# FurkanOM/tf-ssd

Hardware: AMD Instinct MI355X
Metric: images/sec SSD300 (MobileNetV2) fwd+NMS (higher is better)
Workload: dtype f32

## Files before the change

### tf-ssd_amd/csrc/ssd_conv.h

```cpp
#pragma once
#include "common.h"

namespace ssd {

struct ConvParams {
    const float* in;
    const float* w;
    const short* w3;
    const float* scale;
    const float* shift;
    const float* residual;
    float* out;
    int B, H, W, Cin, Ho, Wo, Cout;
    int kh, kw, stride, dil, pad_t, pad_l;
    int K, Kpad, Npad;
    long M;
    long out_batch_stride, out_pixel_stride;
    int n_split;
    float* out2;
    long out2_batch_stride, out2_pixel_stride;
    int vec_store2;
    int act;
    int vec_store;
    int split_k;
    float* partial;
    const float* wino_w;
    int bf16;
    const short* xp;
    long xp_plane;
    int xp_np;
    short* op;
    long op_plane;
    int op_np;
};
bool conv_config_allowed(int cfg, int precision);
inline int conv_vec_store(const ConvParams& p) {
    return (((uintptr_t)p.out & 15) == 0) && (p.out_pixel_stride % 4 == 0) && (p.out_batch_stride % 4 == 0);
}

struct FusedBlockParams {
    const float* x;
    float* y;
    const float* we;
    const float *es, *eh;
    const float* wd;
    const float *ds, *dh;
    const float* wp;
    const float *ps, *ph;
    int residual;
    int B, H, W, Cin, Ce, Cout, Ho, Wo, stride, pad_t, pad_l;
    int kpad_e, kpad_p, npad_p;
    int tiles_y, tiles_x;
    int bf16;
    int groups;
    const short* we3;
    const short* wp3;
    int bands;
    float* slabs;
    unsigned* tickets;
    float* e_out;
    short* y_planes;
    long y_plane;
    short* e_planes;
    long e_plane;
    int planes_np;
    int planes_only;
    int form2;
};
struct StemParams {
    const float* x;
    float* y;
    const float* w1;
    const float *s1, *h1;
    const float* wd;
    const float *sd, *hd;
    const float* wp;
    const float *sp, *hp;
    int B, H, W, H1, W1, pad_t, pad_l, kpad1, kpadp;
    int tiles_y, tiles_x;
    int bf16;
};
struct DwProjParams {
    const float* e;
    const float* wd;
    const float* dh;
    const float* wp;
    const float* ph;
    const float* res;
    float* y;
    int B, H, W, Ce, Cout, Ho, Wo, stride, pad_t, pad_l;
    int kpad_p, npad_p;
    int tiles_y, tiles_x;
    int bf16;
};
bool dwproj_supported(const DwProjParams& p);
int launch_dwproj(DwProjParams p, hipStream_t st);
bool stem_supported(const StemParams& p);
int launch_stem(StemParams p, hipStream_t st);
bool image_block2_supported(const FusedBlockParams& p);
int launch_image_block2(FusedBlockParams p, hipStream_t st);
bool fused_block_supported(const FusedBlockParams& p);
int launch_fused_block(FusedBlockParams p, hipStream_t st);
bool band3_block_supported(const FusedBlockParams& p);
size_t band3_we_shorts(int Ce);
size_t band3_wp_shorts(int npad_p, int Ce);
int launch_band3_pack(const float* we, int Ce, int Cin, int kpad_e, short* we3, const float* wp, int npad_p, int kpad_p,
                      short* wp3, hipStream_t st);
int launch_band3_block(FusedBlockParams p, hipStream_t st);
bool band_block_supported(const FusedBlockParams& p);
int launch_band_block(FusedBlockParams p, hipStream_t st);
bool image_block_supported(const FusedBlockParams& p);
bool image_block_split_fits(FusedBlockParams p);
int image_block_groups(const FusedBlockParams& p, int B);
size_t image_block_slab_floats(const FusedBlockParams& p, int B);
int launch_image_block(FusedBlockParams p, hipStream_t st);

inline int round_up(int v, int a) { return (v + a - 1) / a * a; }
inline int conv_kpad(int K) { return round_up(K, 32); }
inline int conv_npad(int Cout) { return round_up(Cout, 16); }

int conv_num_configs();
const char* conv_config_name(int cfg);
bool conv_config_valid(int cfg, const ConvParams& p);
int conv_pick_config(const ConvParams& p);
long conv_grid_blocks(int cfg, const ConvParams& p);
int conv_k_tiles(int cfg, const ConvParams& p);
int conv_launch(const ConvParams& p, int cfg, hipStream_t st);
size_t conv_splitk_workspace_floats(const ConvParams& p, int cfg);

int fill_conv_params(const ssd_conv_desc* d, ConvParams* p);
int launch_splitk_reduce(const ConvParams& p, hipStream_t st);

int conv_num_mfma_configs();
int wino_num_configs();
const char* wino_config_name(int i);
bool wino_applicable(const ConvParams& p);
bool wino_config_valid(int i, const ConvParams& p);
long wino_grid_blocks(int i, const ConvParams& p);
int wino_k_tiles(const ConvParams& p);
int wino_launch(const ConvParams& p, int i, hipStream_t st);
size_t wino_weight_floats(int Cin, int Cout);
int launch_wino_pack(const float* hwio, int Cin, int Cout, int Npad, int row_off, float* U, hipStream_t st);

int skinny_num_configs();
const char* skinny_config_name(int i);
bool skinny_config_valid(int i, const ConvParams& p);
long skinny_grid_blocks(int i, const ConvParams& p);
int skinny_launch(const ConvParams& p, int i, hipStream_t st);

int mfma3_num_configs();
const char* mfma3_config_name(int i);
bool mfma3_config_valid(int i, const ConvParams& p);
long mfma3_grid_blocks(int i, const ConvParams& p);
int mfma3_k_tiles(const ConvParams& p);
void mfma3_tile(int i, int* BM, int* BN);
int mfma3_launch(const ConvParams& p, int i, hipStream_t st, bool bf16 = false);
const char* bf16_config_name(int i);

int dma_num_configs();
const char* dma_config_name(int i, int np);
bool dma_config_valid(int i, int np, const ConvParams& p);
long dma_grid_blocks(int i, const ConvParams& p);
int dma_k_tiles(int np, const ConvParams& p);
// ... 35 lines not shown
```

### tf-ssd_amd/csrc/ssd_fused.hip

```cpp
#include <cstdlib>

#include "ssd_conv.h"
#include "ssd_bf16x3.h"
#include "ssd_block_common.h"

namespace ssd {

constexpr int kCK = 48;
constexpr int kLDE = kCK + 8;
constexpr int ldx_for(int cinp) { return cinp <= 24 ? 24 : cinp + 4; }

template <int NP, int CINP, int IW, int IPX>
__device__ __forceinline__ void expand_px_tiles(const float* Xs, const float* Wes, float* Es, const float* Ps,
                                                const int Ce, const int ce0, const int pt0, const int pt1,
                                                const int lane, const int iy0, const int ix0, const int H,
                                                const int W) {
    constexpr int LDX = ldx_for(CINP);
    const int frow = lane & 15, fk = (lane >> 4) * 4;
    const int pts[2] = {pt0, pt1};
    f32x4 ea[NP][3];
#pragma unroll
    for (int ct = 0; ct < 3; ++ct) {
        const f32x4 sh = *reinterpret_cast<const f32x4*>(Ps + Ce + ce0 + ct * 16 + (lane >> 4) * 4);
#pragma unroll
// ... 276 lines not shown
        }
    }
}

template <int CINP, int NTC, int S, int TH, int TW>
constexpr size_t fused_static_floats() {
    constexpr int IH = (TH - 1) * S + 3, IW = (TW - 1) * S + 3;
    constexpr int IPXP = (IH * IW + 15) / 16 * 16;
    return (size_t)IPXP * ldx_for(CINP) + (size_t)IPXP * kLDE + (size_t)TH * TW * kLDE + (size_t)kCK * ldx_for(CINP) +
           (size_t)NTC * 16 * kLDE;
}

typedef void (*fused_kernel_t)(const FusedBlockParams);

struct FusedCfg {
    int cinp, ntc, stride, th, tw, res;
    size_t static_floats;
    fused_kernel_t fn;
};
#define FCFG(CINP, NTC, S, TH, TW, RES)                                             \
    {CINP, NTC, S, TH, TW, RES, fused_static_floats<CINP, NTC, S, TH, TW>(),        \
     mbv2_block_kernel<CINP, NTC, S, TH, TW, RES != 0>}
static const FusedCfg kFused[] = {
    FCFG(16, 2, 2, 4, 8, 0),
    FCFG(24, 2, 1, 8, 8, 1),
    FCFG(24, 2, 2, 4, 8, 0),
    FCFG(32, 2, 1, 8, 8, 1),
    FCFG(32, 2, 1, 8, 8, 0),
    FCFG(32, 2, 2, 4, 8, 0),
    FCFG(32, 4, 2, 4, 8, 0),
    FCFG(32, 4, 1, 8, 8, 0),
    FCFG(32, 4, 1, 8, 8, 1),
};

static const FusedCfg* pick_fused(const FusedBlockParams& p) {
    if (p.Ce % kCK != 0 || p.Cin % 4 != 0 || p.Cout % 4 != 0 || p.e_out) return nullptr;
    const int cinp = p.Cin <= 16 ? 16 : (p.Cin == 24 ? 24 : (p.Cin <= 32 ? 32 : 0));
    const int ntc = p.Cout <= 32 ? 2 : (p.Cout <= 64 ? 4 : 0);
    if (!cinp || !ntc) return nullptr;
    for (const auto& c : kFused)
        if (c.cinp == cinp && c.ntc == ntc && c.stride == p.stride && c.res == (p.residual ? 1 : 0)) return &c;
    return nullptr;
}

bool fused_block_supported(const FusedBlockParams& p) { return pick_fused(p) != nullptr; }

int launch_fused_block(FusedBlockParams p, hipStream_t st) {
    const FusedCfg* c = pick_fused(p);
    if (!c) {
        set_error("fused block: unsupported shape Cin=%d Ce=%d Cout=%d stride=%d", p.Cin, p.Ce, p.Cout, p.stride);
        return SSD_E_UNSUPPORTED;
    }
    if (p.B == 0) return SSD_OK;
    p.tiles_y = (p.Ho + c->th - 1) / c->th;
    p.tiles_x = (p.Wo + c->tw - 1) / c->tw;
    const long tiles = (long)p.B * p.tiles_y * p.tiles_x;
    static int num_cu = 0;
    if (!num_cu) {
        int dev = 0;
        (void)hipGetDevice(&dev);
        if (hipDeviceGetAttribute(&num_cu, hipDeviceAttributeMultiprocessorCount, dev) != hipSuccess || num_cu <= 0)
            num_cu = 256;
    }
    constexpr int per_cu = 2;
    const long blocks = tiles < (long)per_cu * num_cu ? tiles : (long)per_cu * num_cu;
    const size_t lds = (c->static_floats + (size_t)13 * p.Ce + (size_t)2 * c->ntc * 16) * sizeof(float);
    SSD_UNSUPPORTED_IF(lds > 160 * 1024, "fused block: needs %zu B of LDS", lds);
    if (lds > 64 * 1024)
        SSD_HIP(hipFuncSetAttribute((const void*)c->fn, hipFuncAttributeMaxDynamicSharedMemorySize, (int)lds));
    hipLaunchKernelGGL(c->fn, dim3((unsigned)blocks), dim3(256), lds, st, p);
    SSD_LAUNCH_CHECK();
    return SSD_OK;
}

constexpr int kSTH = 8, kSTW = 16;
constexpr int kSIH = kSTH + 2, kSIW = kSTW + 2;
constexpr int kSPH = 2 * (kSIH - 1) + 3, kSPW = 2 * (kSIW - 1) + 3;
constexpr int kSLD = 40;
constexpr int kSPQ = (kSPW * 3 + 3 + 3) / 4, kSPR = kSPQ * 4;
constexpr int kSPS = (kSPH * kSPQ + 63) / 64 * 256;

template <bool DMA>
constexpr int stem_patch_floats() { return DMA ? 2 * kSPS : kSPH * kSPW * 3 + 5; }
template <bool DMA>
constexpr int stem_lds_floats() {
    return stem_patch_floats<DMA>() + kSIH * kSIW * kSLD + kSTH * kSTW * kSLD + 27 * 32 + 9 * 32 + 32 * 2 + 32 * 2 + 16 * 2;
}
template <int NP, bool DMA>
__device__ __forceinline__ void stem_body(const StemParams& p, float* __restrict__ sm) {
    static_assert(NP == 1 || NP == 3, "bf16 or split-bf16 operands");
    constexpr int RP = DMA ? kSPR : kSPW * 3;
    float* patch = sm;
    float* C1 = patch + stem_patch_floats<DMA>();
    float* D = C1 + kSIH * kSIW * kSLD;
    float* W1 = D + kSTH * kSTW * kSLD;
    float* Wd = W1 + 27 * 32;
    float* H1 = Wd + 9 * 32;
    float* Hd = H1 + 32;
    float* Hp = Hd + 32;

    const int tid = threadIdx.x, lane = tid & 63, wave = tid >> 6;
    int koff[2][4];
    int kcol[2][4];
    BP<NP> w1b[2], wpb;
    {
        f32x4 wl[2][2];
#pragma unroll
        for (int j = 0; j < 8; ++j) {
            const int k = (lane >> 4) * 8 + j;
            koff[j >> 2][j & 3] = k < 27 ? (k / 9) * RP + (k % 9) : 0;
            kcol[j >> 2][j & 3] = k < 27 ? k % 9 : 0;
#pragma unroll
            for (int ct = 0; ct < 2; ++ct) {
                const int ch = ct * 16 + (lane & 15);
                wl[ct][j >> 2][j & 3] = k < 27 ? p.w1[(long)ch * p.kpad1 + k] * p.s1[ch] : 0.f;
            }
        }
#pragma unroll
        for (int ct = 0; ct < 2; ++ct) w1b[ct] = splitN<NP>(wl[ct][0], wl[ct][1]);
        const int n = lane & 15;
        const float* wr = p.wp + (long)n * p.kpadp + (lane >> 4) * 8;
        f32x4 lo = *reinterpret_cast<const f32x4*>(wr), hi = *reinterpret_cast<const f32x4*>(wr + 4);
        wpb = splitN<NP>(lo * p.sp[n], hi * p.sp[n]);
    }
    for (int e = tid; e < 9 * 32; e += 256) Wd[e] = p.wd[e] * p.sd[e & 31];
    if (tid < 32) { H1[tid] = p.h1[tid]; Hd[tid] = p.hd[tid]; }
    if (tid < 16) Hp[tid] = p.hp[tid];

    const int tiles_per_img = p.tiles_y * p.tiles_x;
    const long total_tiles = (long)p.B * tiles_per_img;
    int du_row[3], du_q[3];
    if (DMA) {
#pragma unroll
        for (int j = 0; j < 3; ++j) {
            const int u = (wave + 4 * j) * 64 + lane;
            du_row[j] = u / kSPQ;
            du_q[j] = u - du_row[j] * kSPQ;
        }
    }
    auto tile_origin = [&](long tile, int& b, int& oy0, int& ox0, int& iy0, int& ix0) {
        b = (int)(tile / tiles_per_img);
        const int rem = (int)(tile - (long)b * tiles_per_img);
        const int ty = rem / p.tiles_x, tx = rem - ty * p.tiles_x;
        oy0 = ty * kSTH; ox0 = tx * kSTW;
        iy0 = (oy0 - 1) * 2 - p.pad_t; ix0 = (ox0 - 1) * 2 - p.pad_l;
    };
    auto issue_patch = [&](long tile, int stage) {
        if constexpr (DMA) {
            int b, oy0, ox0, iy0, ix0;
            tile_origin(tile, b, oy0, ox0, iy0, ix0);
            const __amdgpu_buffer_rsrc_t rs = __builtin_amdgcn_make_buffer_rsrc(const_cast<float*>(p.x + (long)b * p.H * p.W * 3), 0,
                                                                               p.H * p.W * 12, 0x00020000);
            const int fs = ((ix0 * 3) >> 2) * 4;
#pragma unroll
            for (int j = 0; j < 3; ++j) {
                const int ii = __builtin_amdgcn_readfirstlane(wave) + 4 * j;
                if (ii * 64 >= kSPH * kSPQ) continue;
                const int iy = iy0 + du_row[j];
                const bool ok = du_row[j] < kSPH && (unsigned)iy < (unsigned)p.H;
                const int off = ok ? (iy * p.W * 3 + fs + du_q[j] * 4) * 4 : (int)0x80000000;
                __builtin_amdgcn_raw_ptr_buffer_load_lds(rs, (lds_dst_t)(patch + stage * kSPS + ii * 256), 16, off, 0, 0, 0);
            }
        }
    };
    if (DMA && blockIdx.x < total_tiles) {
        issue_patch(blockIdx.x, 0);
        asm volatile("s_waitcnt vmcnt(0)" ::: "memory");
    }
    int it = 0;
    for (long tile = blockIdx.x; tile < total_tiles; tile += gridDim.x, ++it) {
        int b, oy0, ox0, iy0, ix0;
        tile_origin(tile, b, oy0, ox0, iy0, ix0);
        const int cy0 = oy0 - 1, cx0 = ox0 - 1;
        const float* img = p.x + (long)b * p.H * p.W * 3;
        const float* pbuf = patch;
        int psh = 0;

        __syncthreads();
        if constexpr (DMA) {
            pbuf = patch + (it & 1) * kSPS;
            psh = ix0 * 3 - ((ix0 * 3) >> 2) * 4;
            if (tile + gridDim.x < total_tiles) issue_patch(tile + gridDim.x, (it + 1) & 1);
        } else {
        {
            constexpr int NLD = (kSPH * kSPW * 3 + 255) / 256;
            float tmp[NLD];
#pragma unroll
            for (int i = 0; i < NLD; ++i) {
                const int e = tid + i * 256;
                const int r = e / (kSPW * 3), j = e - r * (kSPW * 3);
                const int iy = iy0 + r, ixc = ix0 * 3 + j;
                tmp[i] = 0.f;
                if (e < kSPH * kSPW * 3 && (unsigned)iy < (unsigned)p.H && ixc >= 0 && ixc < p.W * 3)
                    tmp[i] = img[(long)iy * p.W * 3 + ixc];
            }
#pragma unroll
            for (int i = 0; i < NLD; ++i) {
                const int e = tid + i * 256;
                if (e < kSPH * kSPW * 3) patch[e] = tmp[i];
            }
        }
        __syncthreads();
        }
        const int xlim = (p.W - ix0) * 3;
        const bool xedge = DMA && xlim < kSPW * 3;

        {
            constexpr int NHP = kSIH * kSIW;
            int hp[3], rr[3], cc[3];
            const float* pp[3];
            f32x4 a0[3], a1[3];
#pragma unroll
            for (int q = 0; q < 3; ++q) {
                hp[q] = (wave * 3 + q) * 16 + (lane & 15);
                const int hpc = hp[q] < NHP ? hp[q] : NHP - 1;
                rr[q] = hpc / kSIW;
                cc[q] = hpc - rr[q] * kSIW;
                pp[q] = pbuf + (2 * rr[q]) * RP + 2 * cc[q] * 3 + psh;
                a0[q] = *reinterpret_cast<const f32x4*>(H1 + (lane >> 4) * 4);
                a1[q] = *reinterpret_cast<const f32x4*>(H1 + 16 + (lane >> 4) * 4);
            }
#pragma unroll
            for (int q = 0; q < 3; ++q) {
                f32x4 lo, hi;
#pragma unroll
                for (int j = 0; j < 4; ++j) {
                    lo[j] = pp[q][koff[0][j]];
                    hi[j] = pp[q][koff[1][j]];
                }
                if (xedge) {
#pragma unroll
                    for (int j = 0; j < 4; ++j) {
                        if (cc[q] * 6 + kcol[0][j] >= xlim) lo[j] = 0.f;
                        if (cc[q] * 6 + kcol[1][j] >= xlim) hi[j] = 0.f;
                    }
                }
                const BP<NP> b = splitN<NP>(lo, hi);
                a0[q] = mmaN<NP>(w1b[0], b, a0[q]);
                a1[q] = mmaN<NP>(w1b[1], b, a1[q]);
            }
#pragma unroll
            for (int q = 0; q < 3; ++q) {
                const bool in = (unsigned)(cy0 + rr[q]) < (unsigned)p.H1 && (unsigned)(cx0 + cc[q]) < (unsigned)p.W1;
                const float hi = in ? 6.0f : 0.0f;
#pragma unroll
                for (int j = 0; j < 4; ++j) {
                    a0[q][j] = __builtin_amdgcn_fmed3f(a0[q][j], 0.0f, hi);
                    a1[q][j] = __builtin_amdgcn_fmed3f(a1[q][j], 0.0f, hi);
                }
                if (hp[q] < NHP) {
                    *reinterpret_cast<f32x4*>(C1 + hp[q] * kSLD + (lane >> 4) * 4) = a0[q];
                    *reinterpret_cast<f32x4*>(C1 + hp[q] * kSLD + 16 + (lane >> 4) * 4) = a1[q];
                }
            }
        }
        if constexpr (DMA) lds_barrier();
        else __syncthreads();

        {
            const int c4 = (tid & 7) * 4, strip = tid >> 3;
            const int oy = strip >> 2, ox = (strip & 3) * 4;
            f32x4 a[4];
            const f32x4 sh = *reinterpret_cast<const f32x4*>(Hd + c4);
#pragma unroll
            for (int t = 0; t < 4; ++t) a[t] = sh;
#pragma unroll
            for (int ky = 0; ky < 3; ++ky) {
                f32x4 e[6];
#pragma unroll
                for (int j = 0; j < 6; ++j) e[j] = *reinterpret_cast<const f32x4*>(C1 + ((oy + ky) * kSIW + ox + j) * kSLD + c4);
#pragma unroll
                for (int kx = 0; kx < 3; ++kx) {
                    const f32x4 w = *reinterpret_cast<const f32x4*>(Wd + (ky * 3 + kx) * 32 + c4);
#pragma unroll
                    for (int t = 0; t < 4; ++t) {
                        a[t] += e[t + kx] * w;
                    }
                }
            }
#pragma unroll
            for (int t = 0; t < 4; ++t) {
                f32x4 v = a[t];
#pragma unroll
                for (int j = 0; j < 4; ++j) v[j] = relu6f(v[j]);
                *reinterpret_cast<f32x4*>(D + (oy * kSTW + ox + t) * kSLD + c4) = v;
            }
        }
        if constexpr (DMA) lds_barrier();
        else __syncthreads();

        const int frow = lane & 15;
        f32x4 acc[2];
        acc[0] = acc[1] = *reinterpret_cast<const f32x4*>(Hp + (lane >> 4) * 4);
#pragma unroll
        for (int q = 0; q < 2; ++q) {
            const float* dr = D + ((wave + 4 * q) * 16 + frow) * kSLD + (lane >> 4) * 8;
            const BP<NP> b = splitN<NP>(*reinterpret_cast<const f32x4*>(dr), *reinterpret_cast<const f32x4*>(dr + 4));
            acc[q] = mmaN<NP>(wpb, b, acc[q]);
        }
        if constexpr (DMA) asm volatile("s_waitcnt vmcnt(0)" ::: "memory");
#pragma unroll
        for (int q = 0; q < 2; ++q) {
            const int po = (wave + 4 * q) * 16 + (lane & 15);
            const int oy = oy0 + po / kSTW, ox = ox0 + po % kSTW;
            if (oy < p.H1 && ox < p.W1)
                *reinterpret_cast<f32x4*>(p.y + (((long)b * p.H1 + oy) * p.W1 + ox) * 16 + (lane >> 4) * 4) = acc[q];
        }
    }
}

template <int NP, bool DMA>
__global__ __launch_bounds__(256) void mbv2_stem_kernel(const StemParams p) {
    __shared__ __attribute__((aligned(1024))) float sm[stem_lds_floats<DMA>()];
    stem_body<NP, DMA>(p, sm);
}

bool stem_supported(const StemParams& p) { return p.H1 >= 1 && p.W1 >= 1; }

int launch_stem(StemParams p, hipStream_t st) {
    if (p.B == 0) return SSD_OK;
    p.tiles_y = (p.H1 + kSTH - 1) / kSTH;
    p.tiles_x = (p.W1 + kSTW - 1) / kSTW;
    const long tiles = (long)p.B * p.tiles_y * p.tiles_x;
    const long blocks = tiles < 512 ? tiles : 512;
    const bool bf16 = p.bf16 == 1;
    const bool dma = p.W % 4 == 0 && (((uintptr_t)p.x) & 15) == 0 && (long)p.H * p.W * 12 < 0x7fffffffL;
    const auto fn = dma ? (bf16 ? mbv2_stem_kernel<1, true> : mbv2_stem_kernel<3, true>)
                        : (bf16 ? mbv2_stem_kernel<1, false> : mbv2_stem_kernel<3, false>);
    hipLaunchKernelGGL(fn, dim3((unsigned)blocks), dim3(256), 0, st, p);
    SSD_LAUNCH_CHECK();
    return SSD_OK;
}

}
```

### tf-ssd_amd/csrc/ssd_net.h

```cpp
#pragma once
#include <map>
#include <set>
#include <string>
#include <vector>

#include "ssd_conv.h"

struct ssd_train_state;
void ssd_train_state_free(ssd_train_state*);

namespace ssd {

enum LayerKind { LK_CONV = 0, LK_DW, LK_POOL, LK_L2NORM, LK_SOFTMAX, LK_FUSED };
static const char* kKindName[] = {"conv", "dw", "pool", "l2norm", "softmax", "fused"};

enum Route { RT_OFF = 0, RT_LAYER, RT_STEM, RT_DWPROJ, RT_TILE, RT_BAND, RT_BAND3, RT_IMAGE, RT_IMAGE_SPLIT };

struct Param {
    std::string name;
    std::vector<int> shape;
    size_t count = 0;
    float* dev = nullptr;
    bool set = false;
    bool in_flat = false;
// ... 17 lines not shown
    int in = -1, out = -1, res = -1;
    int H = 0, W = 0, Cin = 0, Ho = 0, Wo = 0, Cout = 0;
    int kh = 1, kw = 1, stride = 1, dil = 1, pt = 0, pl = 0, pb = 0, pr = 0, act = 0;
    int p_kernel = -1, p_bias = -1, p_bn = -1;
    int p_kernel2 = -1, p_bias2 = -1, Cout1 = 0;
    int p_gamma = -1;
    int head_kind = 0;
    long head_off = 0, head_bs = 0, head_ps = 0;
    long head2_off = 0, head2_bs = 0, head2_ps = 0;
    float* packed = nullptr;
    float* wino = nullptr;
    float* scale = nullptr;
    float* shift = nullptr;
    int cfg = -1;
    int split_k = 1;
    int f_expand = -1, f_dw = -1, f_project = -1;
    int f_type = 0;
    int fused_by = -1;
    int e_out = -1;
    int img_choice = -1;
    int fused_by2 = -1;
    Route route = RT_OFF;
    float* splitk_part = nullptr;
    float *fz_we = nullptr, *fz_wd = nullptr, *fz_wp = nullptr;
    float *fz_we3 = nullptr, *fz_wp3 = nullptr;
    int side = 0;
    hipEvent_t ev_ready = nullptr;
};

inline void conv_route_head(ConvParams& p, const Layer& l, float* probs, float* deltas) {
    p.out = probs + l.head_off;
    p.out_pixel_stride = l.head_ps;
    p.out_batch_stride = l.head_bs;
    p.n_split = l.Cout1;
    p.out2 = deltas + l.head2_off;
    p.out2_pixel_stride = l.head2_ps;
    p.out2_batch_stride = l.head2_bs;
    p.vec_store2 = (p.out2_pixel_stride % 4 == 0) && (p.out2_batch_stride % 4 == 0);
}

struct ScopedDev {
    float* p = nullptr;
    ~ScopedDev() { if (p) (void)hipFree(p); }
};
struct ScopedEvent {
    hipEvent_t e = nullptr;
    ~ScopedEvent() { if (e) (void)hipEventDestroy(e); }
};

struct Step {
    int layer = -1;
    int sid = -1;
    int wait[2] = {-1, -1};
    bool after_main = false;
    bool publishes = false;
    bool join_first = false;
};

}

struct ssd_net {
    int backbone = 0, img_size = 300, levels = 6, L = 21;
    std::vector<int> n_ars;
    std::vector<ssd::Param> params;
    std::map<std::string, int> param_index;
    std::vector<ssd::Tensor> tensors;
    std::map<std::string, int> tensor_index;
    std::vector<ssd::Layer> layers;
    std::vector<int> fmap;
    std::vector<long> level_off;
    int num_priors = 0;
    bool finalized = false;
    bool fuse_blocks = true;
    bool fuse_softmax = true;
    bool fuse_dwproj = true;
    bool use_wino = true;
    int precision = 0;
    int fuse_band = 2;
    int fuse_image = 1;
    int lanes_hint = 1;
    bool tail_on_side = false;
    bool image_split = true;
    bool image_v2 = true;
    bool conv_dma = true;
    bool plane_only = true;
    bool image_ticket = false;
    float* img_slabs = nullptr;
    unsigned* img_tickets = nullptr;
    int max_batch = 0;
    int last_batch = 0;
    std::vector<float*> owned;
    float* arena = nullptr;
    size_t arena_bytes = 0, plane_bytes = 0, slab_bytes = 0;
    float* splitk_ws = nullptr;
    size_t splitk_floats = 0;
    float* deltas = nullptr;
    float* probs = nullptr;
    void* nms_ws = nullptr;
    size_t nms_ws_bytes = 0;
    int nms_ws_batch = 0;
    int nms_ws_total = 0;
    int scratch_batch = 0;
    std::map<std::string, std::pair<std::string, int>> preset;
    int n_preset = 0;
    int n_autotuned = 0;
    bool launch_raced = false;
    bool use_graph = true;
    bool graphs_unsafe = false;
    bool use_graph_auto = true;
    struct GraphEntry {
        std::vector<const void*> key;
        hipGraphExec_t exec = nullptr;
        hipGraph_t graph = nullptr;
        const float* image = nullptr;
        int batch = 0;
    };
    std::vector<GraphEntry> graphs;
    hipStream_t gstream = nullptr;
    bool overlap_heads = true;
    static constexpr int kSides = 2;
    hipStream_t side[kSides] = {nullptr, nullptr};
    hipEvent_t ev_side_done[kSides] = {nullptr, nullptr};
    std::vector<ssd::Step> steps;
    float* splitk_layers = nullptr;
    bool timing = false;
    ssd_train_state* train = nullptr;
    std::set<std::string> frozen;
    unsigned trainable_rev = 0;
    std::vector<std::vector<hipEvent_t>> timing_events;

    ~ssd_net() {
        for (auto& p : params)
            if (p.dev && !p.in_flat) (void)hipFree(p.dev);
        if (train) ssd_train_state_free(train);
        for (float* p : owned)
            if (p) (void)hipFree(p);
        if (arena) (void)hipFree(arena);
        if (splitk_ws) (void)hipFree(splitk_ws);
        if (deltas) (void)hipFree(deltas);
        if (probs) (void)hipFree(probs);
        if (nms_ws) (void)hipFree(nms_ws);
        for (auto& v : timing_events)
            for (auto e : v) (void)hipEventDestroy(e);
        drop_graphs();
        if (gstream) (void)hipStreamDestroy(gstream);
        for (int k = 0; k < kSides; ++k) {
            if (side[k]) (void)hipStreamDestroy(side[k]);
            if (ev_side_done[k]) (void)hipEventDestroy(ev_side_done[k]);
        }
        for (auto& l : layers)
            if (l.ev_ready) (void)hipEventDestroy(l.ev_ready);
        if (splitk_layers) (void)hipFree(splitk_layers);
    }
    void drop_graphs() {
        steps.clear();
        for (auto& g : graphs) {
            if (g.exec) (void)hipGraphExecDestroy(g.exec);
            if (g.graph) (void)hipGraphDestroy(g.graph);
        }
        graphs.clear();
    }
};
```

### tf-ssd_amd/csrc/ssd_net.hip

```cpp
#include <algorithm>
#include <cstdlib>
#include <cstring>
#include <map>
#include <memory>
#include <string>
#include <vector>

#include "ssd_net.h"

using namespace ssd;

namespace ssd {

struct Builder {
    ssd_net& net;
    explicit Builder(ssd_net& n) : net(n) {}

    int add_param(const std::string& name, std::vector<int> shape) {
        Param p;
        p.name = name;
        p.shape = std::move(shape);
        p.count = 1;
        for (int d : p.shape) p.count *= (size_t)d;
        net.params.push_back(p);
// ... 293 lines not shown
    return p;
}

static FusedBlockParams fused_shape(const ssd_net& net, const Layer& f, int B) {
    const Layer& le = net.layers[f.f_expand];
    const Layer& ld = net.layers[f.f_dw];
    const Layer& lp = net.layers[f.f_project];
    FusedBlockParams p{};
    p.x = net.tensors[f.in].dev;
    p.y = net.tensors[f.out].dev;
    p.we = f.fz_we; p.es = le.scale; p.eh = le.shift;
    p.wd = f.fz_wd; p.ds = ld.scale; p.dh = ld.shift;
    p.wp = f.fz_wp; p.ps = lp.scale; p.ph = lp.shift;
    p.residual = lp.res >= 0 ? 1 : 0;
    p.B = B; p.H = f.H; p.W = f.W; p.Cin = f.Cin; p.Ce = le.Cout; p.Cout = f.Cout;
    p.Ho = f.Ho; p.Wo = f.Wo; p.stride = f.stride; p.pad_t = f.pt; p.pad_l = f.pl;
    p.kpad_e = conv_kpad(le.Cin);
    p.kpad_p = conv_kpad(lp.Cin);
    p.npad_p = conv_npad(lp.Cout);
    p.e_out = f.e_out >= 0 ? net.tensors[f.e_out].dev : nullptr;
    if (f.out >= 0 && net.tensors[f.out].planes_live) {
        const Tensor& to = net.tensors[f.out];
        p.y_planes = to.planes; p.y_plane = to.plane_stride; p.planes_np = to.planes_np;
    }
    if (f.e_out >= 0 && net.tensors[f.e_out].planes_live) {
        const Tensor& te = net.tensors[f.e_out];
        p.e_planes = te.planes; p.e_plane = te.plane_stride; p.planes_np = te.planes_np;
    }
    if (f.route == RT_IMAGE || f.route == RT_IMAGE_SPLIT)
        p.planes_only = (p.y_planes && net.tensors[f.out].plane_only ? 1 : 0) | (p.e_planes && net.tensors[f.e_out].plane_only ? 2 : 0);
    p.we3 = reinterpret_cast<const short*>(f.fz_we3);
    p.wp3 = reinterpret_cast<const short*>(f.fz_wp3);
    p.bf16 = net.precision;
    p.form2 = net.image_v2 ? 1 : 0;
    return p;
}

static FusedBlockParams fused_params(const ssd_net& net, const Layer& f, int B) {
    FusedBlockParams p = fused_shape(net, f, B);
    if (f.route == RT_IMAGE || f.route == RT_IMAGE_SPLIT) {
        const Layer& le = net.layers[f.f_expand];
        const Layer& lp = net.layers[f.f_project];
        p.we3 = conv_split_planes(f.fz_we, le.Cin, le.Cout);
        p.wp3 = conv_split_planes(f.fz_wp, lp.Cin, lp.Cout);
        p.groups = net.img_slabs ? image_block_groups(p, B * net.lanes_hint) : 1;
        p.slabs = net.img_slabs;
        p.tickets = net.image_ticket && !p.bf16 ? net.img_tickets : nullptr;
        if (f.route == RT_IMAGE_SPLIT) { p.bf16 = 3; p.tickets = nullptr; }
    }
    return p;
}

static DwProjParams dwproj_params(const ssd_net& net, const Layer& f, int B) {
    const Layer& ld = net.layers[f.f_dw];
    const Layer& lp = net.layers[f.f_project];
    DwProjParams p{};
    p.e = net.tensors[f.in].dev;
    p.y = net.tensors[f.out].dev;
    p.wd = f.fz_wd; p.dh = ld.shift;
    p.wp = f.fz_wp; p.ph = lp.shift;
    p.res = lp.res >= 0 ? net.tensors[lp.res].dev : nullptr;
    p.B = B; p.H = f.H; p.W = f.W; p.Ce = ld.Cout; p.Cout = f.Cout;
    p.Ho = f.Ho; p.Wo = f.Wo; p.stride = f.stride; p.pad_t = f.pt; p.pad_l = f.pl;
    p.kpad_p = conv_kpad(lp.Cin);
    p.npad_p = conv_npad(lp.Cout);
    p.bf16 = net.precision;
    return p;
}

static StemParams stem_params(const ssd_net& net, const Layer& f, int B) {
    const Layer& l1 = net.layers[f.f_expand];
    const Layer& ld = net.layers[f.f_dw];
    const Layer& lp = net.layers[f.f_project];
    StemParams p{};
    p.x = net.tensors[f.in].dev;
    p.y = net.tensors[f.out].dev;
    p.w1 = l1.packed; p.s1 = l1.scale; p.h1 = l1.shift;
    p.wd = net.params[ld.p_kernel].dev; p.sd = ld.scale; p.hd = ld.shift;
    p.wp = lp.packed; p.sp = lp.scale; p.hp = lp.shift;
    p.B = B; p.H = f.H; p.W = f.W; p.H1 = f.Ho; p.W1 = f.Wo; p.pad_t = f.pt; p.pad_l = f.pl;
    p.kpad1 = conv_kpad(27);
    p.kpadp = conv_kpad(32);
    p.bf16 = net.precision;
    return p;
}

static int planes_pass(ssd_net& net, int tensor, int B, hipStream_t st) {
    Tensor& t = net.tensors[tensor];
    return launch_split_planes(t.dev, (long)B * (long)t.per_image, t.C, t.planes_np, t.planes, t.plane_stride, st);
}

static int run_layer_kernels(ssd_net& net, const Layer& l, int B, float* deltas_out, float* probs_out, hipStream_t st,
                             int cfg_override) {
    const float* in = l.in >= 0 ? net.tensors[l.in].dev : nullptr;
    float* out = l.out >= 0 ? net.tensors[l.out].dev : nullptr;
    switch (l.kind) {
        case LK_CONV: {
            const float* res = l.res >= 0 ? net.tensors[l.res].dev : nullptr;
            ConvParams p = layer_conv_params(net, l, B, in, out, res, deltas_out, probs_out);
            const int cfg = cfg_override >= 0 ? cfg_override : l.cfg;
            const int rc = conv_launch(p, cfg, st);
            if (!rc && p.op && !conv_config_writes_planes(cfg, p)) return planes_pass(net, l.out, B, st);
            return rc;
        }
        case LK_DW:
            return launch_dwconv3x3(in, B, l.H, l.W, l.Cin, l.stride, l.pt, l.pl, l.Ho, l.Wo,
                                    net.params[l.p_kernel].dev, l.scale, l.shift, l.act, out, st);
        case LK_POOL: {
            const Tensor& to = net.tensors[l.out];
            return launch_maxpool(in, B, l.H, l.W, l.Cin, l.kh, l.stride, l.pt, l.pl, l.Ho, l.Wo, to.plane_only ? nullptr : out, st,
                                  to.planes_live ? to.planes : nullptr, to.plane_stride, to.planes_np);
        }
        case LK_L2NORM: {
            const Tensor& to = net.tensors[l.out];
            return launch_l2norm(in, (long)B * l.H * l.W, l.Cin, net.params[l.p_gamma].dev, to.plane_only ? nullptr : out, st,
                                 to.planes_live ? to.planes : nullptr, to.plane_stride, to.planes_np);
        }
        case LK_SOFTMAX:
            return launch_softmax(probs_out, (long)B * net.num_priors, net.L, probs_out, st);
        case LK_FUSED:
            switch (l.route) {
                case RT_STEM: return launch_stem(stem_params(net, l, B), st);
                case RT_DWPROJ: return launch_dwproj(dwproj_params(net, l, B), st);
                case RT_TILE: return launch_fused_block(fused_params(net, l, B), st);
                case RT_BAND: return launch_band_block(fused_params(net, l, B), st);
                case RT_BAND3: return launch_band3_block(fused_params(net, l, B), st);
                case RT_IMAGE:
                case RT_IMAGE_SPLIT: return launch_image_block(fused_params(net, l, B), st);
                default: break;
            }
            set_error("run_layer: no fused kernel is routed to layer %s", l.name.c_str());
            return SSD_E_STATE;
    }
    return SSD_OK;
}

static int run_layer_impl(ssd_net& net, const Layer& l, int B, float* deltas_out, float* probs_out, hipStream_t st,
                          int cfg_override) {
    int rc = run_layer_kernels(net, l, B, deltas_out, probs_out, st, cfg_override);
    if (rc || l.kind == LK_CONV || l.kind == LK_POOL || l.kind == LK_L2NORM || l.kind == LK_SOFTMAX) return rc;
    if ((l.route == RT_IMAGE || l.route == RT_IMAGE_SPLIT) && !net.image_ticket) return rc;
    if (l.out >= 0 && net.tensors[l.out].planes_live) rc = planes_pass(net, l.out, B, st);
    if (!rc && l.kind == LK_FUSED && l.e_out >= 0 && net.tensors[l.e_out].planes_live) rc = planes_pass(net, l.e_out, B, st);
    return rc;
}

static int run_layer(ssd_net& net, const Layer& l, int B, float* deltas_out, float* probs_out, hipStream_t st,
                     int cfg_override = -1) {
    static const bool dbg_sync = getenv("SSD_HIP_DEBUG_SYNC") != nullptr;
    if (!dbg_sync) return run_layer_impl(net, l, B, deltas_out, probs_out, st, cfg_override);
    fprintf(stderr, "[ssd dbg] run %s\n", l.name.c_str());
    const int rc = run_layer_impl(net, l, B, deltas_out, probs_out, st, cfg_override);
    hipStreamCaptureStatus cs = hipStreamCaptureStatusNone;
    (void)hipStreamIsCapturing(st, &cs);
    if (!rc && cs == hipStreamCaptureStatusNone) SSD_HIP(hipStreamSynchronize(st));
    return rc;
}

static bool image_kernel_takes(const FusedBlockParams& p) { return !fused_block_supported(p) && image_block_supported(p); }
static bool image_kernel_takes(const ssd_net& net, const Layer& f) {
    return f.kind == LK_FUSED && f.f_type == 0 && image_kernel_takes(fused_shape(net, f, 1));
}

static Route fused_route(const ssd_net& net, const Layer& f) {
    if (!net.fuse_blocks) return RT_OFF;
    if (f.f_type == 1) return stem_supported(stem_params(net, f, 1)) ? RT_STEM : RT_OFF;
// ... 904 lines not shown
                    float* scores_dev, int* valid_dev, void* stream) {
    SSD_CHECK_ARG(net != nullptr, "ssd_net_predict: net is NULL");
    if (!net->finalized) {
        set_error("ssd_net_predict: call ssd_net_finalize() first");
        return SSD_E_STATE;
    }
    const int N = net->num_priors, L = net->L;
    SSD_CHECK_ARG(B >= 0 && B <= net->max_batch, "ssd_net_predict: batch %d exceeds max_batch %d", B, net->max_batch);
    SSD_CHECK_ARG(max_total >= 1, "ssd_net_predict: max_total must be >= 1");
    if (net->scratch_batch < net->max_batch) {
        (void)hipDeviceSynchronize();
        net->drop_graphs();
        if (net->deltas) (void)hipFree(net->deltas);
        if (net->probs) (void)hipFree(net->probs);
        net->deltas = net->probs = nullptr;
        net->scratch_batch = 0;
        SSD_HIP(hipMalloc((void**)&net->deltas, (size_t)net->max_batch * N * 4 * sizeof(float)));
        SSD_HIP(hipMalloc((void**)&net->probs, (size_t)net->max_batch * N * L * sizeof(float)));
        net->scratch_batch = net->max_batch;
    }
    const int ws_batch = std::max(net->max_batch, net->nms_ws_batch);
    const size_t need = ssd_decode_nms_workspace_bytes(ws_batch, N, L, max_total);
    if (need > net->nms_ws_bytes || ws_batch != net->nms_ws_batch || max_total != net->nms_ws_total) {
        (void)hipDeviceSynchronize();
        net->drop_graphs();
        if (net->nms_ws) (void)hipFree(net->nms_ws);
        net->nms_ws = nullptr;
        net->nms_ws_bytes = 0;
        SSD_HIP(hipMalloc(&net->nms_ws, need));
        SSD_HIP(hipMemset(net->nms_ws, 0, need));
        net->nms_ws_bytes = need;
        net->nms_ws_batch = ws_batch;
        net->nms_ws_total = max_total;
    }
    hipStream_t st = (hipStream_t)stream;
    SSD_CHECK_ARG(var != nullptr, "ssd_net_predict: variances pointer is NULL");
    const float v4[4] = {var[0], var[1], var[2], var[3]};
    union { float f; intptr_t i; } k1{}, k2{};
    k1.f = iou_thr; k2.f = score_thr;
    std::vector<const void*> key = {image_dev, priors_dev, boxes_dev, labels_dev, scores_dev, valid_dev,
                                    (const void*)(intptr_t)B, (const void*)(intptr_t)max_total,
                                    (const void*)k1.i, (const void*)k2.i, (const void*)2};
    for (int i = 0; i < 4; ++i) { union { float f; intptr_t i; } k{}; k.f = v4[i]; key.push_back((const void*)k.i); }
    const bool fused_sm = net->fuse_softmax && decode_nms_fused_ok(L) && N >= 1 && net->nms_ws_batch >= B;
    int rc = run_graphed(net, key, st, [&]() {
        int r = forward_impl(net, image_dev, B, net->deltas, net->probs, st, fused_sm);
        if (r) return r;
        if (fused_sm)
            return decode_nms_fused(net->deltas, net->probs, priors_dev, v4, B, N, L, max_total, max_total, iou_thr, score_thr,
                                    boxes_dev, labels_dev, scores_dev, valid_dev, net->nms_ws, net->nms_ws_bytes, net->nms_ws_batch, st);
        return ssd_decode_nms(net->deltas, net->probs, priors_dev, v4, B, N, L, max_total, max_total, iou_thr,
                              score_thr, boxes_dev, labels_dev, scores_dev, valid_dev, nullptr, net->nms_ws,
                              net->nms_ws_bytes, (void*)st);
    });
    if (rc && fused_sm && net->nms_ws) {
        (void)hipDeviceSynchronize();
        (void)hipMemset(net->nms_ws, 0, net->nms_ws_bytes);
    }
    if (!rc && net->timing && !net->timing_events.empty())
        (void)hipEventRecord(net->timing_events.back().back(), st);
    return rc;
}

struct OptionSpec {
    const char* name;
    bool ssd_net::*flag;
    int ssd_net::*num;
    int lo, hi, refinalize;
};
static const OptionSpec kOptions[] = {
    {"fuse_blocks", &ssd_net::fuse_blocks, nullptr, 0, 1, 0},
    {"precision", nullptr, &ssd_net::precision, 0, 1, 1},
    {"fuse_band", nullptr, &ssd_net::fuse_band, 0, 2, 0},
    {"fuse_image", nullptr, &ssd_net::fuse_image, 0, 2, 0},
    {"lanes_hint", nullptr, &ssd_net::lanes_hint, 1, 8, 0},
    {"tail_on_side", &ssd_net::tail_on_side, nullptr, 0, 1, 0},
    {"image_split", &ssd_net::image_split, nullptr, 0, 1, 1},
    {"image_ticket", &ssd_net::image_ticket, nullptr, 0, 1, 0},
    {"fuse_softmax", &ssd_net::fuse_softmax, nullptr, 0, 1, 0},
    {"fuse_dwproj", &ssd_net::fuse_dwproj, nullptr, 0, 1, 0},
    {"overlap_heads", &ssd_net::overlap_heads, nullptr, 0, 1, 0},
    {"use_wino", &ssd_net::use_wino, nullptr, 0, 1, 2},
    {"image_v2", &ssd_net::image_v2, nullptr, 0, 1, 0},
    {"conv_dma", &ssd_net::conv_dma, nullptr, 0, 1, 1},
    {"plane_only", &ssd_net::plane_only, nullptr, 0, 1, 0},
    {"use_graph", &ssd_net::use_graph, nullptr, 0, 1, 0},
};

int ssd_net_set_option(ssd_net* net, const char* name, int value) {
    SSD_CHECK_ARG(net && name, "ssd_net_set_option: NULL argument");
    const std::string n(name);
    const OptionSpec* o = nullptr;
    for (const OptionSpec& k : kOptions)
        if (n == k.name) o = &k;
    if (!o) {
        set_error("ssd_net_set_option: unknown option '%s'", name);
        return SSD_E_INVALID;
    }
    if (n == "precision") SSD_CHECK_ARG(value == 0 || value == 1, "ssd_net_set_option: precision must be 0 (fp32) or 1 (bf16)");
    if (n == "use_graph") {
        if (value && net->graphs_unsafe && net->overlap_heads) {
            set_error("ssd_net_set_option: use_graph 1 needs overlap_heads 0 with GPU_MAX_HW_QUEUES < 4 (hipGraph capture of the forked step crashes in the runtime; a single in-order stream replays fine)");
            return SSD_E_UNSUPPORTED;
        }
        net->use_graph_auto = false;
    }
    const int v = o->flag ? value != 0 : std::min(std::max(value, o->lo), o->hi);
    const int old = o->flag ? (int)(net->*o->flag) : net->*o->num;
    if (o->flag) net->*o->flag = v != 0;
    else net->*o->num = v;
    if (o->refinalize == 2 || (o->refinalize == 1 && v != old)) net->finalized = false;
    net->drop_graphs();
    resolve_routes(*net);
    if (n == "fuse_softmax" && net->nms_ws) {
        (void)hipDeviceSynchronize();
        SSD_HIP(hipMemset(net->nms_ws, 0, net->nms_ws_bytes));
    }
    return SSD_OK;
}

int ssd_net_set_timing(ssd_net* net, int enabled) {
    SSD_CHECK_ARG(net != nullptr, "ssd_net_set_timing: net is NULL");
    net->timing = enabled != 0;
    net->steps.clear();
    return SSD_OK;
}

int ssd_net_read_timing(ssd_net* net, float* ms_sum_out, int* forwards_out) {
    SSD_CHECK_ARG(net && ms_sum_out && forwards_out, "ssd_net_read_timing: NULL argument");
    const size_t nl = net->layers.size();
    for (size_t i = 0; i <= nl; ++i) ms_sum_out[i] = 0.f;
    SSD_HIP(hipDeviceSynchronize());
    for (auto& ev : net->timing_events) {
        for (size_t i = 0; i < nl; ++i) {
            float ms = 0.f;
            if (hipEventElapsedTime(&ms, ev[i], ev[i + 1]) == hipSuccess) ms_sum_out[i] += ms;
        }
        float ms = 0.f;
        if (hipEventQuery(ev[nl + 1]) == hipSuccess && hipEventElapsedTime(&ms, ev[nl], ev[nl + 1]) == hipSuccess)
            ms_sum_out[nl] += ms;
        for (auto e : ev) (void)hipEventDestroy(e);
    }
    *forwards_out = (int)net->timing_events.size();
    net->timing_events.clear();
    return SSD_OK;
}

long ssd_net_fetch_activation(ssd_net* net, const char* layer, float* host_out, size_t cap) {
    if (!net || !layer) return SSD_E_INVALID;
    auto it = net->tensor_index.find(layer);
    if (it == net->tensor_index.end()) {
        set_error("ssd_net_fetch_activation: unknown tensor '%s'", layer);
        return SSD_E_INVALID;
    }
    const Tensor& t = net->tensors[it->second];
    const size_t n = t.per_image * (size_t)net->last_batch;
    if (!host_out) return (long)n;
    if (cap < n) {
        set_error("ssd_net_fetch_activation: buffer holds %zu floats, need %zu", cap, n);
        return SSD_E_INVALID;
    }
    ScopedDev joined;
    const float* src = t.dev;
    if (t.plane_only && n) {
        SSD_HIP(hipMalloc((void**)&joined.p, n * sizeof(float)));
        SSD_HIP(hipDeviceSynchronize());
// ... 129 lines not shown
```

Before: 58800.

## Fuse stem depthwise conv into MFMA operand build and size grid by occupancy

Adds a stem kernel form in which each wave computes the depthwise 3x3 output directly in registers, in the layout the projection MFMA needs. This removes the D staging buffer in LDS and the barrier between the depthwise and projection stages. The smaller LDS footprint allows launch bounds of three workgroups per CU, and the grid is now sized from an occupancy query instead of a fixed 512 blocks. The cost is some redundant per-lane depthwise work and higher register pressure.

```diff
diff --git a/tf-ssd_amd/csrc/ssd_conv.h b/tf-ssd_amd/csrc/ssd_conv.h
--- a/tf-ssd_amd/csrc/ssd_conv.h
+++ b/tf-ssd_amd/csrc/ssd_conv.h
@@ -79,6 +79,7 @@
     int B, H, W, H1, W1, pad_t, pad_l, kpad1, kpadp;
     int tiles_y, tiles_x;
     int bf16;
+    int form;
 };
 struct DwProjParams {
     const float* e;
diff --git a/tf-ssd_amd/csrc/ssd_fused.hip b/tf-ssd_amd/csrc/ssd_fused.hip
--- a/tf-ssd_amd/csrc/ssd_fused.hip
+++ b/tf-ssd_amd/csrc/ssd_fused.hip
@@ -382,19 +382,18 @@
 
 template <bool DMA>
 constexpr int stem_patch_floats() { return DMA ? 2 * kSPS : kSPH * kSPW * 3 + 5; }
-template <bool DMA>
+template <bool DMA, int FORM>
 constexpr int stem_lds_floats() {
-    return stem_patch_floats<DMA>() + kSIH * kSIW * kSLD + kSTH * kSTW * kSLD + 27 * 32 + 9 * 32 + 32 * 2 + 32 * 2 + 16 * 2;
-}
-template <int NP, bool DMA>
+    return stem_patch_floats<DMA>() + kSIH * kSIW * kSLD + (FORM ? 0 : kSTH * kSTW * kSLD) + 9 * 32 + 32 + 32 + 16;
+}
+template <int NP, bool DMA, int FORM>
 __device__ __forceinline__ void stem_body(const StemParams& p, float* __restrict__ sm) {
     static_assert(NP == 1 || NP == 3, "bf16 or split-bf16 operands");
     constexpr int RP = DMA ? kSPR : kSPW * 3;
     float* patch = sm;
     float* C1 = patch + stem_patch_floats<DMA>();
     float* D = C1 + kSIH * kSIW * kSLD;
-    float* W1 = D + kSTH * kSTW * kSLD;
-    float* Wd = W1 + 27 * 32;
+    float* Wd = D + (FORM ? 0 : kSTH * kSTW * kSLD);
     float* H1 = Wd + 9 * 32;
     float* Hd = H1 + 32;
     float* Hp = Hd + 32;
@@ -557,51 +556,81 @@
         if constexpr (DMA) lds_barrier();
         else __syncthreads();
 
-        {
-            const int c4 = (tid & 7) * 4, strip = tid >> 3;
-            const int oy = strip >> 2, ox = (strip & 3) * 4;
-            f32x4 a[4];
-            const f32x4 sh = *reinterpret_cast<const f32x4*>(Hd + c4);
-#pragma unroll
-            for (int t = 0; t < 4; ++t) a[t] = sh;
-#pragma unroll
-            for (int ky = 0; ky < 3; ++ky) {
-                f32x4 e[6];
-#pragma unroll
-                for (int j = 0; j < 6; ++j) e[j] = *reinterpret_cast<const f32x4*>(C1 + ((oy + ky) * kSIW + ox + j) * kSLD + c4);
-#pragma unroll
-                for (int kx = 0; kx < 3; ++kx) {
-                    const f32x4 w = *reinterpret_cast<const f32x4*>(Wd + (ky * 3 + kx) * 32 + c4);
-#pragma unroll
-                    for (int t = 0; t < 4; ++t) {
-                        a[t] += e[t + kx] * w;
-                    }
-                }
-            }
-#pragma unroll
-            for (int t = 0; t < 4; ++t) {
-                f32x4 v = a[t];
-#pragma unroll
-                for (int j = 0; j < 4; ++j) v[j] = relu6f(v[j]);
-                *reinterpret_cast<f32x4*>(D + (oy * kSTW + ox + t) * kSLD + c4) = v;
-            }
-        }
-        if constexpr (DMA) lds_barrier();
-        else __syncthreads();
-
-        const int frow = lane & 15;
         f32x4 acc[2];
         acc[0] = acc[1] = *reinterpret_cast<const f32x4*>(Hp + (lane >> 4) * 4);
+        if constexpr (FORM) {
+            const int c8 = (lane >> 4) * 8;
+            const float* cr = C1 + (2 * wave * kSIW + (lane & 15)) * kSLD + c8;
+            f32x4 d[2][2];
+            d[0][0] = d[1][0] = *reinterpret_cast<const f32x4*>(Hd + c8);
+            d[0][1] = d[1][1] = *reinterpret_cast<const f32x4*>(Hd + c8 + 4);
+#pragma unroll
+            for (int ky = 0; ky < 3; ++ky)
+#pragma unroll
+                for (int kx = 0; kx < 3; ++kx) {
+                    const f32x4 w0 = *reinterpret_cast<const f32x4*>(Wd + (ky * 3 + kx) * 32 + c8);
+                    const f32x4 w1 = *reinterpret_cast<const f32x4*>(Wd + (ky * 3 + kx) * 32 + c8 + 4);
+#pragma unroll
+                    for (int q = 0; q < 2; ++q) {
+                        const float* er = cr + ((q + ky) * kSIW + kx) * kSLD;
+                        d[q][0] += *reinterpret_cast<const f32x4*>(er) * w0;
+                        d[q][1] += *reinterpret_cast<const f32x4*>(er + 4) * w1;
+                    }
+                }
+#pragma unroll
+            for (int q = 0; q < 2; ++q) {
+#pragma unroll
+                for (int j = 0; j < 4; ++j) {
+                    d[q][0][j] = relu6f(d[q][0][j]);
+                    d[q][1][j] = relu6f(d[q][1][j]);
+                }
+                acc[q] = mmaN<NP>(wpb, splitN<NP>(d[q][0], d[q][1]), acc[q]);
+            }
+        } else {
+            {
+                const int c4 = (tid & 7) * 4, strip = tid >> 3;
+                const int oy = strip >> 2, ox = (strip & 3) * 4;
+                f32x4 a[4];
+                const f32x4 sh = *reinterpret_cast<const f32x4*>(Hd + c4);
+#pragma unroll
+                for (int t = 0; t < 4; ++t) a[t] = sh;
+#pragma unroll
+                for (int ky = 0; ky < 3; ++ky) {
+                    f32x4 e[6];
+#pragma unroll
+                    for (int j = 0; j < 6; ++j) e[j] = *reinterpret_cast<const f32x4*>(C1 + ((oy + ky) * kSIW + ox + j) * kSLD + c4);
+#pragma unroll
+                    for (int kx = 0; kx < 3; ++kx) {
+                        const f32x4 w = *reinterpret_cast<const f32x4*>(Wd + (ky * 3 + kx) * 32 + c4);
+#pragma unroll
+                        for (int t = 0; t < 4; ++t) {
+                            a[t] += e[t + kx] * w;
+                        }
+                    }
+                }
+#pragma unroll
+                for (int t = 0; t < 4; ++t) {
+                    f32x4 v = a[t];
+#pragma unroll
+                    for (int j = 0; j < 4; ++j) v[j] = relu6f(v[j]);
+                    *reinterpret_cast<f32x4*>(D + (oy * kSTW + ox + t) * kSLD + c4) = v;
+                }
+            }
+            if constexpr (DMA) lds_barrier();
+            else __syncthreads();
+
+            const int frow = lane & 15;
+#pragma unroll
+            for (int q = 0; q < 2; ++q) {
+                const float* dr = D + ((wave + 4 * q) * 16 + frow) * kSLD + (lane >> 4) * 8;
+                const BP<NP> b = splitN<NP>(*reinterpret_cast<const f32x4*>(dr), *reinterpret_cast<const f32x4*>(dr + 4));
+                acc[q] = mmaN<NP>(wpb, b, acc[q]);
+            }
+        }
+        if constexpr (DMA) asm volatile("s_waitcnt vmcnt(0)" ::: "memory");
 #pragma unroll
         for (int q = 0; q < 2; ++q) {
-            const float* dr = D + ((wave + 4 * q) * 16 + frow) * kSLD + (lane >> 4) * 8;
-            const BP<NP> b = splitN<NP>(*reinterpret_cast<const f32x4*>(dr), *reinterpret_cast<const f32x4*>(dr + 4));
-            acc[q] = mmaN<NP>(wpb, b, acc[q]);
-        }
-        if constexpr (DMA) asm volatile("s_waitcnt vmcnt(0)" ::: "memory");
-#pragma unroll
-        for (int q = 0; q < 2; ++q) {
-            const int po = (wave + 4 * q) * 16 + (lane & 15);
+            const int po = (FORM ? 2 * wave + q : wave + 4 * q) * 16 + (lane & 15);
             const int oy = oy0 + po / kSTW, ox = ox0 + po % kSTW;
             if (oy < p.H1 && ox < p.W1)
                 *reinterpret_cast<f32x4*>(p.y + (((long)b * p.H1 + oy) * p.W1 + ox) * 16 + (lane >> 4) * 4) = acc[q];
@@ -609,24 +638,39 @@
     }
 }
 
-template <int NP, bool DMA>
-__global__ __launch_bounds__(256) void mbv2_stem_kernel(const StemParams p) {
-    __shared__ __attribute__((aligned(1024))) float sm[stem_lds_floats<DMA>()];
-    stem_body<NP, DMA>(p, sm);
+template <int NP, bool DMA, int FORM>
+__global__ __launch_bounds__(256, FORM ? 3 : 1) void mbv2_stem_kernel(const StemParams p) {
+    __shared__ __attribute__((aligned(1024))) float sm[stem_lds_floats<DMA, FORM>()];
+    stem_body<NP, DMA, FORM>(p, sm);
 }
 
 bool stem_supported(const StemParams& p) { return p.H1 >= 1 && p.W1 >= 1; }
+
+typedef void (*stem_kernel_t)(const StemParams);
+#define STEM_FORMS(NP, DMA) {mbv2_stem_kernel<NP, DMA, 0>, mbv2_stem_kernel<NP, DMA, 1>}
+static const stem_kernel_t kStem[2][2][2] = {{STEM_FORMS(3, false), STEM_FORMS(3, true)},
+                                             {STEM_FORMS(1, false), STEM_FORMS(1, true)}};
 
 int launch_stem(StemParams p, hipStream_t st) {
     if (p.B == 0) return SSD_OK;
     p.tiles_y = (p.H1 + kSTH - 1) / kSTH;
     p.tiles_x = (p.W1 + kSTW - 1) / kSTW;
     const long tiles = (long)p.B * p.tiles_y * p.tiles_x;
-    const long blocks = tiles < 512 ? tiles : 512;
-    const bool bf16 = p.bf16 == 1;
-    const bool dma = p.W % 4 == 0 && (((uintptr_t)p.x) & 15) == 0 && (long)p.H * p.W * 12 < 0x7fffffffL;
-    const auto fn = dma ? (bf16 ? mbv2_stem_kernel<1, true> : mbv2_stem_kernel<3, true>)
-                        : (bf16 ? mbv2_stem_kernel<1, false> : mbv2_stem_kernel<3, false>);
+    const int bf16 = p.bf16 == 1;
+    const int dma = p.W % 4 == 0 && (((uintptr_t)p.x) & 15) == 0 && (long)p.H * p.W * 12 < 0x7fffffffL;
+    const int form = p.form != 0;
+    const stem_kernel_t fn = kStem[bf16][dma][form];
+    static int resident[2][2][2];
+    int& grid = resident[bf16][dma][form];
+    if (!grid) {
+        int dev = 0, num_cu = 0, per_cu = 0;
+        SSD_HIP(hipGetDevice(&dev));
+        SSD_HIP(hipDeviceGetAttribute(&num_cu, hipDeviceAttributeMultiprocessorCount, dev));
+        SSD_HIP(hipOccupancyMaxActiveBlocksPerMultiprocessor(&per_cu, (const void*)fn, 256, 0));
+        SSD_UNSUPPORTED_IF(num_cu <= 0 || per_cu <= 0, "stem: the occupancy query gave %d CUs x %d workgroups", num_cu, per_cu);
+        grid = num_cu * per_cu;
+    }
+    const long blocks = tiles < grid ? tiles : grid;
     hipLaunchKernelGGL(fn, dim3((unsigned)blocks), dim3(256), 0, st, p);
     SSD_LAUNCH_CHECK();
     return SSD_OK;
diff --git a/tf-ssd_amd/csrc/ssd_net.h b/tf-ssd_amd/csrc/ssd_net.h
--- a/tf-ssd_amd/csrc/ssd_net.h
+++ b/tf-ssd_amd/csrc/ssd_net.h
@@ -123,6 +123,7 @@
     bool tail_on_side = false;
     bool image_split = true;
     bool image_v2 = true;
+    bool stem_form = true;
     bool conv_dma = true;
     bool plane_only = true;
     bool image_ticket = false;
diff --git a/tf-ssd_amd/csrc/ssd_net.hip b/tf-ssd_amd/csrc/ssd_net.hip
--- a/tf-ssd_amd/csrc/ssd_net.hip
+++ b/tf-ssd_amd/csrc/ssd_net.hip
@@ -399,6 +399,7 @@
     p.kpad1 = conv_kpad(27);
     p.kpadp = conv_kpad(32);
     p.bf16 = net.precision;
+    p.form = net.stem_form ? 1 : 0;
     return p;
 }
 
@@ -1469,6 +1470,7 @@
     {"overlap_heads", &ssd_net::overlap_heads, nullptr, 0, 1, 0},
     {"use_wino", &ssd_net::use_wino, nullptr, 0, 1, 2},
     {"image_v2", &ssd_net::image_v2, nullptr, 0, 1, 0},
+    {"stem_form", &ssd_net::stem_form, nullptr, 0, 1, 0},
     {"conv_dma", &ssd_net::conv_dma, nullptr, 0, 1, 1},
     {"plane_only", &ssd_net::plane_only, nullptr, 0, 1, 0},
     {"use_graph", &ssd_net::use_graph, nullptr, 0, 1, 0},
```

New measurement: 59310 (median of 6 runs). About the same (+0.9%).
